# stormalex/minimap2_chaindp

Measured on AMD Instinct MI355X. Metric: chained anchors/sec (whole node), higher is better.
Workload: dtype int32

## Files before the change

### minimap2_chaindp_amd/csrc/chaindp_twin.hip

```cpp
#include <hip/hip_runtime.h>
#include <stdint.h>
#include <limits.h>
#include <stdio.h>
#include <stdlib.h>
#include <vector>
#include "chaindp_kernels.h"
#include "chaindp_wave.h"
#include "chaindp_lanes.h"

namespace chaindp {

#define TW_XY 0u
#define TW_PF 2048u
#define TW_V 3072u
#define TW_LUT_BYTES 512u
#define TW_ST_HALF 56u
#define TW_MK_HALF 260u
template <bool ONE_LUT> struct TwLayout {
	static constexpr bool HAS_XQ = !ONE_LUT;
	static constexpr uint32_t XQ = 3584u, XQ_HALF = 512u;
	static constexpr uint32_t LUT = ONE_LUT ? 3584u : XQ + 2u * XQ_HALF;
	static constexpr uint32_t LUT_HALF = ONE_LUT ? 0u : TW_LUT_BYTES;
	static constexpr uint32_t ST = LUT + (ONE_LUT ? 1u : 2u) * TW_LUT_BYTES;
	static constexpr uint32_t MK = ST + 2u * TW_ST_HALF;
	static constexpr uint32_t SP = MK + 2u * TW_MK_HALF;
	static constexpr uint32_t SP_HALF = ONE_LUT ? 0u : 64u;
	static constexpr uint32_t SP_OF_XQ = SP - XQ / 8u;
	static constexpr uint32_t KEY = SP + 128u;
	static constexpr uint32_t KEY_HALF = ONE_LUT ? 0u : 4u;
	static constexpr uint32_t BYTES = KEY + 8u;
	static_assert(ST % 8u == 0u && MK % 4u == 0u && KEY % 4u == 0u, "cold state is read as 64-bit words, marks and keys as 32-bit");
};
static_assert(TwLayout<true>::BYTES == 4864u && TwLayout<true>::BYTES <= 5120u, "one table: 32 workgroups per CU");
static_assert(TwLayout<false>::BYTES == 6400u, "two tables: 24 workgroups per CU");
template <bool SAMEGAP, bool ONE_LUT> struct TwWaves { static constexpr int N = !ONE_LUT ? 6 : SAMEGAP ? 8 : 7; };
#define TW_TILE 64
#define TW_RING 64
#define TW_QCH 8

__device__ __forceinline__ int tw_excl_max32(int v)
{
	v = max(v, __builtin_amdgcn_update_dpp(0, v, DPP_ROW_SHR(1), 0xf, 0xf, true));
	v = max(v, __builtin_amdgcn_update_dpp(0, v, DPP_ROW_SHR(2), 0xf, 0xf, true));
	v = max(v, __builtin_amdgcn_update_dpp(0, v, DPP_ROW_SHR(4), 0xf, 0xf, true));
	v = max(v, __builtin_amdgcn_update_dpp(0, v, DPP_ROW_SHR(8), 0xf, 0xf, true));
	int e = __builtin_amdgcn_update_dpp(0, v, DPP_ROW_SHR(1), 0xf, 0xf, true);
#if defined(__HIP_DEVICE_COMPILE__)
	asm("s_nop 1\n\tv_max_i32_dpp %0, %1, %0 row_bcast:15 row_mask:0xa bank_mask:0xf" : "+v"(e) : "v"(v));
#endif
	return e;
}
__device__ __forceinline__ int tw_incl_min32(int v)
{
	v = min(v, dpp_or_old<DPP_ROW_SHR(1), 0xf>(INT_MAX, v));
	v = min(v, dpp_or_old<DPP_ROW_SHR(2), 0xf>(INT_MAX, v));
	v = min(v, dpp_or_old<DPP_ROW_SHR(4), 0xf>(INT_MAX, v));
	v = min(v, dpp_or_old<DPP_ROW_SHR(8), 0xf>(INT_MAX, v));
	v = min(v, dpp_or_old<DPP_ROW_BCAST15, 0xa>(INT_MAX, v));
	return v;
}

__device__ __forceinline__ int tw_below_in_half(uint64_t m, bool hi_half)
{
	const int lo = (int)__builtin_amdgcn_mbcnt_lo((uint32_t)m, 0u);
	const int hi = (int)__builtin_amdgcn_mbcnt_hi((uint32_t)(m >> 32), 0u);
	return hi_half ? hi : lo;
}

__device__ __forceinline__ uint64_t tw_smear_halves(uint64_t m)
{
	uint32_t lo = 0, hi = 0;
#if defined(__HIP_DEVICE_COMPILE__)
	asm("s_cmp_lg_u32 %2, 0\n\ts_cselect_b32 %0, -1, 0\n\ts_cmp_lg_u32 %3, 0\n\ts_cselect_b32 %1, -1, 0"
	    : "=&s"(lo), "=&s"(hi) : "s"(TW_UNI((uint32_t)m)), "s"(TW_UNI((uint32_t)(m >> 32))) : "scc");
#endif
	return (uint64_t)hi << 32 | lo;
}

__device__ __forceinline__ uint64_t tw_last_or_lane0(uint64_t m)
{
	uint32_t lo = 0, hi = 0;
#if defined(__HIP_DEVICE_COMPILE__)
	asm("s_flbit_i32_b32 %0, %2\n\ts_flbit_i32_b32 %1, %3\n\ts_lshr_b32 %0, 0x80000000, %0\n\ts_lshr_b32 %1, 0x80000000, %1"
	    : "=&s"(lo), "=&s"(hi) : "s"(TW_UNI((uint32_t)m)), "s"(TW_UNI((uint32_t)(m >> 32))));
#endif
	return (uint64_t)hi << 32 | lo;
}

__device__ __forceinline__ uint32_t tw_both_halves(uint64_t m)
{
	uint32_t t = 0;
#if defined(__HIP_DEVICE_COMPILE__)
	asm("s_cmp_lg_u32 %1, 0\n\ts_cselect_b32 %0, %2, 0" : "=s"(t) : "s"(TW_UNI((uint32_t)m)), "s"(TW_UNI((uint32_t)(m >> 32))) : "scc");
#endif
	return t;
}

__device__ __forceinline__ uint64_t tw_below_first(uint64_t m, uint64_t b)
{
	const uint32_t blo = (uint32_t)b, bhi = (uint32_t)(b >> 32);
	const uint32_t klo = blo ? (blo & (0u - blo)) - 1u : 0xffffffffu, khi = bhi ? (bhi & (0u - bhi)) - 1u : 0xffffffffu;
	return m & ((uint64_t)khi << 32 | klo);
}

#define TW_HI31 0x8000000080000000ull

__device__ __forceinline__ uint64_t tw_above_first(uint64_t a, uint64_t b)
{
	uint32_t lo = 0, hi = 0;
#if defined(__HIP_DEVICE_COMPILE__)
	asm("s_sub_i32 %0, 0, %2\n\ts_sub_i32 %1, 0, %3" : "=&s"(lo), "=&s"(hi) : "s"(TW_UNI((uint32_t)b)), "s"(TW_UNI((uint32_t)(b >> 32))) : "scc");
#endif
	return a & ((uint64_t)hi << 32 | lo);
}

__device__ __forceinline__ void tw_st64_pf_lanes(uint64_t m, uint32_t a, uint32_t x, uint32_t y)
{
#if defined(__HIP_DEVICE_COMPILE__)
	tw_u32x2 t; t.x = x; t.y = y;
	uint64_t saved;
	asm volatile("s_and_saveexec_b64 %0, %1\n\tds_write_b64 %2, %3 offset:2048\n\ts_mov_b64 exec, %0"
	             : "=&s"(saved) : "s"(m), "v"(a), "v"(t) : "memory", "scc");
#endif
}
static_assert(TW_PF == 2048u, "tw_st64_pf_lanes writes the PF ring at DS offset 2048");


struct TwinArgs {
	Params par;
	const int64_t *off;
	const ulonglong2 *a;
	const unsigned long long *sumq;
	const uint16_t *lut;
	int lut_stride;
	const Unit *units;
	const UnitAux *aux;
	const unsigned long long *counters;
	int32_t *f, *p, *v;
	int32_t *first_child;
	uint8_t *flags;
	Unit *left;
	unsigned int *left_cnt;
	unsigned int *queue;
	const unsigned int *key_range;
	unsigned int *route;
	int two_tables;
	int force_left;
	int64_t total;
	unsigned long long *stamp;
};

struct TwinCold {
	int64_t next;
	int64_t base;
	uint64_t x_carry;
	int32_t rel0, room, read, tile0;
};

struct TwinHot {
	uint32_t S;
	uint32_t m4;
	uint32_t pc;
	uint32_t pend;
};
#define TW_CARRY 40u

#ifdef CHAINDP_TWIN_STAMPS
#define TW_STAMP(...) __VA_ARGS__
#else
#define TW_STAMP(...)
#endif
#if defined(CHAINDP_TWIN_STAMPS) && CHAINDP_TWIN_STAMPS == 2
#define TW_STAMP_A(...)
#define TW_STAMP_B(...) __VA_ARGS__
#elif defined(CHAINDP_TWIN_STAMPS) && CHAINDP_TWIN_STAMPS == 1
#define TW_STAMP_A(...) __VA_ARGS__
#define TW_STAMP_B(...)
#else
#define TW_STAMP_A(...)
#define TW_STAMP_B(...)
#endif
#if defined(CHAINDP_TWIN_STAMPS) && CHAINDP_TWIN_STAMPS == 3
#define TW_STAMP_C(...) __VA_ARGS__
#else
#define TW_STAMP_C(...)
#endif
#define TW_NOW() __builtin_amdgcn_s_memtime()

template <bool SAMEGAP, bool ONE_LUT>
__global__ __launch_bounds__(64) __attribute__((amdgpu_waves_per_eu(TwWaves<SAMEGAP, ONE_LUT>::N, TwWaves<SAMEGAP, ONE_LUT>::N))) void k_chain_twin(TwinArgs g)
{
	using L = TwLayout<ONE_LUT>;
	const int lane = threadIdx.x;
	const bool hi_half = lane >= 32;
	const int h = lane >> 5, hl = lane & 31;

	uint32_t L16 = ((uint32_t)hl + 1u) << 4;
	const uint32_t mkbase = L::MK + TW_MK_HALF * (uint32_t)h;
	const uint32_t curbase = L::XQ + L::XQ_HALF * (uint32_t)h;
	uint32_t c_mkbase = mkbase;
	uint32_t c_far = mkbase + 256u;
	uint32_t c_own = mkbase + ((uint32_t)hl << 2);
	uint32_t c_lut = ONE_LUT ? 0u : L::LUT + L::LUT_HALF * (uint32_t)h;
	uint32_t c_8h = (uint32_t)h << 3;
	uint32_t c_M = (uint32_t)g.par.max_dist_x;
	uint32_t c_bw = (uint32_t)g.par.bw;
	uint32_t c_cbw = c_M - 1u > c_bw ? c_M - 1u - c_bw : 0u;
	const uint32_t mdq = (uint32_t)(g.par.max_dist_x < g.par.max_dist_y ? g.par.max_dist_x : g.par.max_dist_y);
	uint32_t c_dqoff = c_M - mdq;
	int c_ms = g.par.max_skip;
	int c_min = INT_MIN;
	int c_Mout = hl == 31 ? g.par.max_dist_x : INT_MAX;
	uint32_t c_bwl = c_bw + c_lut;
	uint32_t c_cbwl = c_cbw - c_lut;
	constexpr uint32_t LUT_OFF = ONE_LUT ? L::LUT : 0u;
	TW_VREG(L16); TW_VREG(c_far); TW_VREG(c_own);
	if (!ONE_LUT) { TW_VREG(c_M); TW_VREG(c_ms); }
	if (!ONE_LUT) TW_VREG(c_lut);
	if (!SAMEGAP) TW_VREG(c_dqoff);
	TW_VREG(c_min); TW_VREG(c_Mout); TW_VREG(c_bwl); TW_VREG(c_cbwl);

	const uint64_t maxx = (uint64_t)(int64_t)g.par.max_dist_x;
	const uint32_t route = *g.route;
	if (ONE_LUT ? route == 1u || g.key_range[0] != g.key_range[1] || g.two_tables : route == 1u || route == 2u) return;
	const int64_t n_units = (int64_t)(uint32_t)g.counters[0];
	const int64_t n_single = (int64_t)(g.counters[0] >> 32);
	const bool short_units = (g.total - n_single) <= 512 * n_units;
	if (!short_units) {
		if (blockIdx.x == 0 && lane == 0) *g.left_cnt = 0xffffffffu;
		return;
	}
	if (blockIdx.x == 0 && lane == 0) *g.route = ONE_LUT ? 2u : 3u;
	const bool params_ok = g.lut != nullptr && !g.par.is_cdna && g.par.max_dist_x >= 1 && g.par.max_dist_y >= 0 &&
	                       ((uint64_t)(int64_t)g.par.max_dist_x + 1) * 129ull < (1ull << 31) && g.par.bw + 1 <= (int)TW_LUT_BYTES && g.force_left != 1;

	TwinHot u;
	u.S = 0; u.m4 = 0; u.pc = L::HAS_XQ ? curbase : 0u; u.pend = u.pc;
	uint64_t live_m = ~0ull;
	uint64_t contm = 0;
	const uint32_t st_addr = L::ST + TW_ST_HALF * (uint32_t)h;
#define TW_COLD (*TW_LDS(TwinCold, st_addr))
	const uint32_t xcd = blockIdx.x & 7u;
	const uint32_t n_halves = 2u * gridDim.x;
#ifndef TW_END_UNITS
#define TW_END_UNITS 16u
#define TW_PIECE 1u
#endif
	const uint32_t U1 = n_units > (long long)TW_END_UNITS * n_halves ? ((uint32_t)n_units - TW_END_UNITS * n_halves) & ~(8u * TW_QCH - 1u) : 0u;
	const uint32_t G1k = U1 / (8u * TW_QCH);
	auto grab = [&](uint32_t p, uint32_t &nx, uint32_t &ne) {
		if (p < G1k) { nx = (8u * p + xcd) * TW_QCH; ne = nx + TW_QCH; }
		else { nx = U1 + TW_PIECE * (8u * (p - G1k) + xcd); ne = nx + TW_PIECE; }
	};
	if (hl == 0) {
		uint32_t nx, ne;
		grab(((blockIdx.x >> 3) << 1) | (uint32_t)h, nx, ne);
		tw_st64(st_addr, nx, ne); tw_st64(st_addr + 8u, 0u, 0u);
		tw_st64(st_addr + 16u, 0u, 0u); tw_st64(st_addr + 24u, 0u, 0u);
		tw_st64(st_addr + 32u, 0u, (uint32_t)-TW_TILE);
		tw_st64(st_addr + TW_CARRY, 0xfffffffcu, 0u); tw_st64(st_addr + TW_CARRY + 8u, 0u, 0u);
		tw_st32(L::KEY + 4u * (uint32_t)h, -1);
	}
	wave_mem_fence();

	constexpr bool PF = !ONE_LUT;
	uint64_t nx0_x = 0, nx0_y = 0, nx1_x = 0, nx1_y = 0;
	int32_t pfu0 = -1, pfu1 = -1;

	TW_STAMP(unsigned long long st_t0 = 0; unsigned int st_service = 0, st_n_service = 0, st_n_fast = 0, st_flush = 0, st_unit = 0, st_n_unit = 0, st_head = 0, st_take = 0, st_tail = 0;)

	auto service = [&](uint64_t svc) {
#if defined(__HIP_DEVICE_COMPILE__)
		asm volatile("s_waitcnt vmcnt(0)" ::: "memory");
#endif
		wave_mem_fence();
		uint64_t retired = 0;
		for (int hs = 0; hs < 2; ++hs) {
			if (((svc >> (32 * hs)) & 1ull) == 0) continue;
			TW_STAMP_B(const unsigned long long th0 = g.stamp ? TW_NOW() : 0;)
			const uint64_t hm = hs ? 0xffffffff00000000ull : 0x00000000ffffffffull;
			const uint32_t sa = L::ST + TW_ST_HALF * (uint32_t)hs, keya = L::KEY + L::KEY_HALF * (uint32_t)hs;
			const uint32_t mkb = L::MK + TW_MK_HALF * (uint32_t)hs, lutb = L::LUT + L::LUT_HALF * (uint32_t)hs;
			const uint32_t curb = L::XQ + L::XQ_HALF * (uint32_t)hs, spb = L::SP + L::SP_HALF * (uint32_t)hs;
			const tw_u32x2 cw0 = tw_ld64(sa), cw1 = tw_ld64(sa + 8u), cw2 = tw_ld64(sa + 16u), cw3 = tw_ld64(sa + 24u), cw4 = tw_ld64(sa + 32u);
			int64_t c_next = (int64_t)((uint64_t)TW_UNI(cw0.y) << 32 | TW_UNI(cw0.x));
			int64_t c_base = (int64_t)((uint64_t)TW_UNI(cw1.y) << 32 | TW_UNI(cw1.x));
			uint64_t c_xcarry = (uint64_t)TW_UNI(cw2.y) << 32 | TW_UNI(cw2.x);
			int c_rel0 = (int)TW_UNI(cw3.x), c_room = (int)TW_UNI(cw3.y), c_read = (int)TW_UNI(cw4.x), c_tile0 = (int)TW_UNI(cw4.y);
			auto tile_cnt = [&]() -> int {
				const uint32_t pe = TW_UNI(__builtin_amdgcn_readlane((int)u.pend, 32 * hs));
				if constexpr (L::HAS_XQ) return (int)((pe - curb) >> 3);
				else return pe < mkb ? 0 : (int)((pe - mkb) >> 2) + 1 - c_tile0;
			};
			const int cnt_prev = tile_cnt();
			const int slow_h = (int)TW_UNI((uint32_t)tw_ld32(sa + TW_CARRY + 12u));
			const uint32_t cur_key = TW_UNI((uint32_t)tw_ld32(keya));
			const int tile_prev = c_tile0, rel0_prev = c_rel0;
			const int64_t base_prev = c_base;
			bool live = true;
			const uint32_t nx0 = (uint32_t)c_next, ne0 = (uint32_t)((uint64_t)c_next >> 32);
			tw_u32x4 rec0 = {0u, 0u, 0u, 0u}, aux0 = {0u, 0u, 0u, 0u}, rec1 = {0u, 0u, 0u, 0u};
			const bool rec0_ok = nx0 < ne0 && (int64_t)nx0 < n_units;
			const bool rec1_ok = PF && rec0_ok && nx0 + 1u < ne0 && (int64_t)nx0 + 1 < n_units;
			if (rec0_ok) { rec0 = *TW_CONST(tw_u32x4, g.units + nx0); aux0 = *TW_CONST(tw_u32x4, g.aux + nx0); }
			if (rec1_ok) rec1 = *TW_CONST(tw_u32x4, g.units + nx0 + 1u);

			auto take_tile = [&](const uint64_t an_x, const uint64_t an_y) -> int {
				const int i_lane = c_tile0 + lane;
				const bool have = i_lane < c_room;
				uint64_t xp;
				{
					uint32_t lo = (uint32_t)wave_shift_up1((int)(uint32_t)an_x, 0), hi = (uint32_t)wave_shift_up1((int)(uint32_t)(an_x >> 32), 0);
					if (lane == 0) { lo = (uint32_t)c_xcarry; hi = (uint32_t)(c_xcarry >> 32); }
					xp = (uint64_t)hi << 32 | lo;
				}
				const bool stop = !have || (i_lane > 0 && an_x - xp > maxx);
				const uint64_t stop_m = __builtin_amdgcn_ballot_w64(stop);
				const int cnt = stop_m ? __builtin_ctzll(stop_m) : TW_TILE;
				c_xcarry = readlane_u64(an_x, 63);
				if constexpr (L::HAS_XQ) { u.pc = TW_SEL(hm, curb, u.pc); u.pend = TW_SEL(hm, curb + ((uint32_t)cnt << 3), u.pend); }
				else u.pend = TW_SEL(hm, mkb + ((uint32_t)(c_tile0 + cnt - 1) << 2), u.pend);
				if (cnt == 0) return 0;
				wave_mem_fence();
				if (lane < cnt) {
					const int sp = span_of_hi((uint32_t)(an_y >> 32));
					tw_st64((((uint32_t)i_lane & 127u) << 4 | (uint32_t)hs << 3) + TW_XY, (uint32_t)an_x + 1u, (uint32_t)an_y + 1u);
					if constexpr (L::HAS_XQ) {
						tw_st64(curb + ((uint32_t)lane << 3), (uint32_t)an_x, (uint32_t)an_y);
						tw_st8(spb + (uint32_t)lane, sp - 1);
					} else tw_st8((((uint32_t)i_lane & 63u) << 1 | (uint32_t)hs) + L::SP, sp - 1);
					g.first_child[c_base + i_lane] = NO_CHILD;
				}
				wave_mem_fence();
				if constexpr (PF) {
					if (cnt == TW_TILE && c_tile0 + TW_TILE < c_room) {
						uint64_t rx = 0, ry = 0;
						if (i_lane + TW_TILE < c_room) { const ulonglong2 t = g.a[c_base + i_lane + TW_TILE]; rx = t.x; ry = t.y; }
						if (hs) { nx1_x = rx; nx1_y = ry; pfu1 = -1; } else { nx0_x = rx; nx0_y = ry; pfu0 = -1; }
					}
				}
				return cnt;
			};

			bool goes_on = cnt_prev == TW_TILE && c_tile0 + TW_TILE < c_room;
			if (goes_on && (slow_h * 8 > c_tile0 + TW_TILE || g.force_left == 2)) {
				if (lane == 0) {
					Unit un; un.start = (int64_t)((uint64_t)c_base | (uint64_t)(uint32_t)(c_tile0 + TW_TILE) << 32); un.read = c_read; un.len = c_room;
					g.left[atomicAdd(g.left_cnt, 1u)] = un;
				}
				goes_on = false;
			}
			if (goes_on) {
				c_tile0 += TW_TILE;
				uint64_t nt_x = 0, nt_y = 0;
				if constexpr (PF) { nt_x = hs ? nx1_x : nx0_x; nt_y = hs ? nx1_y : nx0_y; }
				else if (c_tile0 + lane < c_room) { const ulonglong2 t = g.a[c_base + c_tile0 + lane]; nt_x = t.x; nt_y = t.y; }
				if (take_tile(nt_x, nt_y) == 0) goes_on = false;
			}
			TW_STAMP_B(if (g.stamp) st_take += (unsigned int)(TW_NOW() - th0);)
			TW_STAMP_A(const unsigned long long tf0 = g.stamp ? TW_NOW() : 0;)
			if (cnt_prev > 0) {
				const int i_lane = tile_prev + lane;
				const bool have = lane < cnt_prev;
				const int64_t gi = base_prev + i_lane;
				int fi = 0, p4 = -4;
				if (have) {
					const tw_u32x2 pf = tw_ld64((((uint32_t)i_lane & 63u) << 4 | (uint32_t)hs << 3) + TW_PF);
					p4 = (int)pf.x; fi = (int)pf.y + 1;
				}
				const int pi = p4 >> 2;
				int val = fi, ptr = have ? pi : -1;
				const bool ext = ptr >= 0 && ptr < tile_prev;
				int vext = 0;
				if (ext) {
					vext = tw_ld32((((uint32_t)ptr & 63u) << 3 | (uint32_t)hs << 2) + TW_V);
					val = max(val, vext & 0x7fffffff);
					ptr = -1;
				}
				const bool ext_self = ext && vext < 0;
				for (int r = 0; r < 6; ++r) {
					if (__builtin_amdgcn_ballot_w64(ptr >= tile_prev) == 0) break;
					const int src = (ptr >= tile_prev ? ptr - tile_prev : lane) << 2;
					const int pv = __builtin_amdgcn_ds_bpermute(src, val);
					const int pp = __builtin_amdgcn_ds_bpermute(src, ptr);
					if (ptr >= tile_prev) { val = max(val, pv); ptr = pp; }
				}
				const bool self = val >= g.par.min_sc || pi >= 0;
				const int srcp = (pi >= tile_prev ? pi - tile_prev : lane) << 2;
				const int pself_in = __builtin_amdgcn_ds_bpermute(srcp, self ? 1 : 0);
				const bool pred_self = ext ? ext_self : pself_in != 0;
				wave_mem_fence();
				if (have) tw_st32((((uint32_t)i_lane & 63u) << 3 | (uint32_t)hs << 2) + TW_V, val | (self ? INT_MIN : 0));
				wave_mem_fence();
				if (have) {
					g.f[gi] = fi;
					g.p[gi] = pi < 0 ? -1 : pi + rel0_prev;
					g.v[gi] = val;
					int maybe_first = 0;
					if (pi >= 0 && !pred_self) { atomicMin(&g.first_child[base_prev + pi], rel0_prev + i_lane); maybe_first = 4; }
					g.flags[gi] = (uint8_t)((self ? 2 : 0) | maybe_first | (val >= g.par.min_sc ? 8 : 0) | (fi < val ? 16 : 0));
				}
			}
			TW_STAMP_A(if (g.stamp) st_flush += (unsigned int)(TW_NOW() - tf0);)
			TW_STAMP_A(const unsigned long long tu0 = g.stamp ? TW_NOW() : 0;)
			TW_STAMP_A(if (g.stamp && !goes_on) ++st_n_unit;)
			bool have_rec = rec0_ok;
			const bool rec0_used = !goes_on;
			uint32_t cur_key_now = cur_key;
			while (!goes_on && live) {
				uint32_t nx = (uint32_t)c_next, ne = (uint32_t)((uint64_t)c_next >> 32);
				if (nx >= ne) {
					uint32_t q0 = 0;
					if (lane == 0) q0 = atomicAdd(g.queue + 64u * xcd, 1u);
					grab(TW_UNI(q0), nx, ne);
					have_rec = false;
				}
				if ((int64_t)nx >= n_units) {
					c_next = (int64_t)((uint64_t)ne << 32 | nx); live = false;
					if constexpr (L::HAS_XQ) { u.pc = TW_SEL(hm, curb, u.pc); u.pend = TW_SEL(hm, curb, u.pend); }
					else u.pend = TW_SEL(hm, 0u, u.pend);
					break;
				}
				TW_STAMP_C(const unsigned long long tc0 = g.stamp ? TW_NOW() : 0;)
				if (!have_rec) { rec0 = *TW_CONST(tw_u32x4, g.units + nx); aux0 = *TW_CONST(tw_u32x4, g.aux + nx); }
				have_rec = false;
				TW_STAMP_C(if (g.stamp) { asm volatile("" :: "s"(rec0.x), "s"(aux0.x)); st_head += (unsigned int)(TW_NOW() - tc0); })
				c_next = (int64_t)((uint64_t)ne << 32 | (nx + 1u));
				Unit un;
				un.start = (int64_t)((uint64_t)rec0.y << 32 | rec0.x); un.read = (int32_t)rec0.z; un.len = (int32_t)rec0.w;
				if (!params_ok || (aux0.z & 1u) || g.par.n_segs > 1 || (ONE_LUT && cur_key_now != 0xffffffffu && aux0.y != cur_key_now)) {
					if (lane == 0) g.left[atomicAdd(g.left_cnt, 1u)] = un;
					continue;
				}
				c_base = un.start; c_rel0 = (int)aux0.x; c_room = un.len; c_read = un.read; c_tile0 = 0;
				uint64_t tl_x = 0, tl_y = 0;
				TW_STAMP_C(const unsigned long long tc1 = g.stamp ? TW_NOW() : 0;)
				TW_STAMP_C(if (g.stamp && PF && (hs ? pfu1 : pfu0) == (int32_t)c_base) ++st_n_unit;)
				if (PF && (hs ? pfu1 : pfu0) == (int32_t)c_base) { tl_x = hs ? nx1_x : nx0_x; tl_y = hs ? nx1_y : nx0_y; }
				else if (lane < c_room) { const ulonglong2 t = g.a[c_base + lane]; tl_x = t.x; tl_y = t.y; }
				if constexpr (PF) { if (hs) pfu1 = -1; else pfu0 = -1; }
				TW_STAMP_C(if (g.stamp) { asm volatile("" :: "v"(tl_x), "v"(tl_y)); asm volatile("s_waitcnt vmcnt(0)" ::: "memory"); st_take += (unsigned int)(TW_NOW() - tc1); })
				TW_STAMP_C(const unsigned long long tc2 = g.stamp ? TW_NOW() : 0;)
				wave_mem_fence();
				if (aux0.y != cur_key_now) {
					const uint2 *src = (const uint2*)(g.lut + (int64_t)c_read * g.lut_stride);
					for (int k = lane; k * 4 <= g.par.bw; k += 64) {
						const uint2 t = src[k];
						const uint32_t w = (t.x & 0xffu) | (t.x >> 8 & 0xff00u) | (t.y << 16 & 0xff0000u) | (t.y << 8 & 0xff000000u);
						tw_st32(lutb + ((uint32_t)k << 2), (int)w);
					}
					cur_key_now = aux0.y;
					if (lane == 0) tw_st32(keya, (int)cur_key_now);
				}
				const uint32_t x_none = (uint32_t)__builtin_amdgcn_readlane((int)(uint32_t)tl_x, 0) - (uint32_t)maxx - 1u;
				for (int k = lane; k < 128; k += 64) tw_st64(((uint32_t)k << 4 | (uint32_t)hs << 3) + TW_XY, x_none, 0u);
				for (int k = lane; k < 65; k += 64) tw_st32(mkb + ((uint32_t)k << 2), -1);
				wave_mem_fence();
				c_xcarry = 0;
				if (lane == 0) tw_st32(sa + TW_CARRY + 12u, 0);
				if (take_tile(tl_x, tl_y) > 0) goes_on = true;
				TW_STAMP_C(if (g.stamp) { st_tail += (unsigned int)(TW_NOW() - tc2); ++st_unit; })
			}
			if (PF && live) {
				const int cnt_now = tile_cnt();
				const uint32_t nxn = (uint32_t)c_next, nen = (uint32_t)((uint64_t)c_next >> 32);
				if (!(cnt_now == TW_TILE && c_tile0 + TW_TILE < c_room) && (hs ? pfu1 : pfu0) < 0 && nxn < nen && (int64_t)nxn < n_units &&
				    ((nxn == nx0 && rec0_ok && !rec0_used) || (nxn == nx0 + 1u && rec1_ok))) {
					const tw_u32x4 rn = nxn == nx0 ? rec0 : rec1;
					const int32_t st = (int32_t)rn.x, ln = (int32_t)rn.w;
					uint64_t rx = 0, ry = 0;
					if (lane < ln) { const ulonglong2 t = g.a[(int64_t)st + lane]; rx = t.x; ry = t.y; }
					if (hs) { nx1_x = rx; nx1_y = ry; pfu1 = st; } else { nx0_x = rx; nx0_y = ry; pfu0 = st; }
				}
			}
			TW_STAMP_A(if (g.stamp) st_unit += (unsigned int)(TW_NOW() - tu0);)
			if (live) {
				const uint32_t i = (uint32_t)c_tile0;
				u.S = TW_SEL(hm, (i - 1u) << 4 | (uint32_t)hs << 3, u.S); u.m4 = TW_SEL(hm, ((i - 1u) << 2) + mkb, u.m4);
			} else retired |= hm;
			if (lane == 0) {
				tw_st64(sa, (uint32_t)c_next, (uint32_t)((uint64_t)c_next >> 32)); tw_st64(sa + 8u, (uint32_t)c_base, (uint32_t)((uint64_t)c_base >> 32));
				tw_st64(sa + 16u, (uint32_t)c_xcarry, (uint32_t)(c_xcarry >> 32)); tw_st64(sa + 24u, (uint32_t)c_rel0, (uint32_t)c_room);
				tw_st64(sa + 32u, (uint32_t)c_read, (uint32_t)c_tile0);
			}
		}
		wave_mem_fence();
		live_m &= ~retired;
		contm &= ~svc;
	};

	auto slow_tail = [&](uint64_t D, uint32_t a_cur, int nskip_after) -> uint64_t {
		const uint64_t giveup = ~D & contm;
		const int vlast = __builtin_amdgcn_ds_bpermute(((h << 5) + 31) << 2, nskip_after);
		wave_mem_fence();
		const tw_u32x2 cur = tw_ld64(a_cur);
		if (__builtin_amdgcn_inverse_ballot_w64(D)) {
			u.m4 += 4u;
			u.S = ((u.m4 - c_mkbase) << 2) | c_8h;
			if constexpr (L::HAS_XQ) u.pc += 8u;
		} else {
			if (hl == 0) {
				tw_st64(st_addr + TW_CARRY, cur.x, cur.y);
				tw_st32(st_addr + TW_CARRY + 8u, vlast);
				tw_st32(st_addr + TW_CARRY + 12u, tw_ld32(st_addr + TW_CARRY + 12u) + 1);
			}
			u.S -= 512u;
		}
		contm = ~D & ~giveup & live_m;
		if (__builtin_expect(giveup != 0, 0)) {
			if (__builtin_amdgcn_inverse_ballot_w64(giveup)) {
				wave_mem_fence();
				if (hl == 0) {
					const TwinCold c = TW_COLD;
					Unit un; un.start = (int64_t)((uint64_t)c.base | (uint64_t)(uint32_t)c.tile0 << 32); un.read = c.read; un.len = c.room;
					g.left[atomicAdd(g.left_cnt, 1u)] = un;
				}
				u.pc = curbase; u.pend = L::HAS_XQ ? curbase : 0u;
			}
			return giveup;
		}
		return 0;
	};

	TW_STAMP(if (g.stamp) st_t0 = TW_NOW();)
	service(~0ull);
	bool force_general = false;
	while (live_m != 0) {
		wave_mem_fence();
		uint64_t svc = 0;
		if (__builtin_expect(contm == 0 && live_m == ~0ull && !force_general, 1)) {
			if constexpr (ONE_LUT) {
				uint64_t B, D = 0;
				bool tile_end = false;
				int npass = 1;
				if constexpr (L::HAS_XQ) {
					const int n0 = (int)(TW_UNI(__builtin_amdgcn_readlane((int)u.pend, 0)) - TW_UNI(__builtin_amdgcn_readlane((int)u.pc, 0))) >> 3;
					const int n1 = (int)(TW_UNI(__builtin_amdgcn_readlane((int)u.pend, 32)) - TW_UNI(__builtin_amdgcn_readlane((int)u.pc, 32))) >> 3;
					npass = max(min(n0, n1), 1);
				} else {
					const int n0 = (int)(TW_UNI(__builtin_amdgcn_readlane((int)u.pend, 0)) - TW_UNI(__builtin_amdgcn_readlane((int)u.m4, 0))) >> 2;
					const int n1 = (int)(TW_UNI(__builtin_amdgcn_readlane((int)u.pend, 32)) - TW_UNI(__builtin_amdgcn_readlane((int)u.m4, 32))) >> 2;
					npass = max(min(n0, n1), 1);
				}
				const uint32_t ms0 = (uint32_t)max(g.par.max_skip, 0);
				u.S += 16u;
				for (;;) {
					const uint32_t S1 = u.S;
					const uint32_t t0 = S1 - L16;
					const tw_u32x2 xy = tw_ld64((t0 & 0x7f8u) + TW_XY);
					const tw_u32x2 cur = tw_ld64(L::HAS_XQ ? u.pc : (S1 & 0x7f8u) + TW_XY);
	#if defined(__HIP_DEVICE_COMPILE__)
					__builtin_amdgcn_sched_barrier(0);
	#endif
					const tw_u32x2 pf = tw_ld64((t0 & 0x3f8u) + TW_PF);
					uint32_t a_cur = S1 & 0x3f8u;
					TW_OPAQUE(a_cur);
					const int spm1 = tw_ld_u8(L::HAS_XQ ? (u.pc >> 3) + L::SP_OF_XQ : (a_cur >> 3) + L::SP);
	#ifdef TW_EXP_PAD
					for (int k = 0; k < TW_EXP_PAD; ++k) { uint32_t pad; asm volatile("v_max3_u32 %0, %1, %1, %1" : "=v"(pad) : "v"(c_far)); }
	#endif
					const uint32_t drm1 = L::HAS_XQ ? cur.x - xy.x : tw_sub_m1(cur.x, xy.x), dqm1 = L::HAS_XQ ? cur.y - xy.y : tw_sub_m1(cur.y, xy.y);
					const uint32_t ddl = ONE_LUT ? tw_absdiff(drm1, dqm1) : tw_sad(drm1, dqm1, c_lut);
					const uint32_t dqs = SAMEGAP ? dqm1 : __builtin_elementwise_add_sat(dqm1, c_dqoff);
					const uint32_t m3 = max(max(drm1, dqs), ddl + c_cbwl);
					const uint64_t okm = TW_ULT(m3, c_M);
					const uint32_t dst = TW_SEL(okm, min(u.m4 - pf.x, c_far), c_far);
					tw_st32(dst, (int)u.m4);
					wave_mem_fence();
					const int tj = tw_ld32(c_own);
					const int lutv = tw_ld_i8(min(ddl, c_bwl) + LUT_OFF);
	#if defined(__HIP_DEVICE_COMPILE__)
					__builtin_amdgcn_sched_barrier(0);
	#endif
					const int sc0 = min(min((int)dqm1, (int)drm1), spm1);
					const int sc = TW_SEL(okm, sc0 + (int)pf.y + lutv, c_min);
					const int excl = max(tw_excl_max32(sc), spm1);
					const uint64_t A = TW_SGT(sc, excl);
					B = TW_EQ(tj, u.m4) & okm & ~A;
					const uint32_t blo = (uint32_t)B, bhi = (uint32_t)(B >> 32);
					if (__builtin_expect(tw_above_first(A, B) != 0, 0)) { force_general = true; break; }
					{
						const uint32_t wp = TW_SEL(A, u.m4 - c_own, 0xfffffffcu);
						const int wf = max(excl, sc);
						tw_st64_pf_lanes(tw_last_or_lane0(A), a_cur, wp, (uint32_t)wf);
					}
					const uint32_t nlo = (uint32_t)__builtin_popcount(blo), nhi = (uint32_t)__builtin_popcount(bhi);
					if (__builtin_expect(min(nlo, nhi) <= ms0, 0)) {
						const uint64_t OUT = TW_SGE(drm1, c_Mout);
						D = tw_smear_halves(OUT | (nlo > ms0 ? 0x00000000ffffffffull : 0ull) | (nhi > ms0 ? 0xffffffff00000000ull : 0ull));
						if (__builtin_expect(tw_both_halves(D) == 0, 0)) break;
					}
					u.m4 += 4u; u.S += 16u;
					if constexpr (L::HAS_XQ) u.pc += 8u;
					TW_STAMP(if (g.stamp) ++st_n_fast;)
					if (__builtin_expect(--npass <= 0, 0)) { tile_end = true; break; }
					wave_mem_fence();
				}
				const uint32_t a_cur = u.S & 0x3f8u;
				u.S -= 16u;
				if (!force_general && !tile_end) {
					svc = slow_tail(D, a_cur + TW_PF, tw_below_in_half(B, hi_half) + (int)__builtin_amdgcn_inverse_ballot_w64(B));
				}
			} else {
				uint64_t B, X, tile;
				int cB;
				uint32_t a_cur;
				for (;;) {
					const uint32_t S1 = u.S + 16u;
					const uint32_t t0 = S1 - L16;
					const tw_u32x2 xy = tw_ld64((t0 & 0x7f8u) + TW_XY);
					const tw_u32x2 cur = tw_ld64(u.pc);
	#if defined(__HIP_DEVICE_COMPILE__)
					__builtin_amdgcn_sched_barrier(0);
	#endif
					const tw_u32x2 pf = tw_ld64((t0 & 0x3f8u) + TW_PF);
					const int spm1 = tw_ld_u8((u.pc >> 3) + L::SP_OF_XQ);
					const uint32_t drm1 = cur.x - xy.x, dqm1 = cur.y - xy.y;
					const uint32_t ddl = tw_sad(drm1, dqm1, c_lut);
					const uint32_t dqs = SAMEGAP ? dqm1 : __builtin_elementwise_add_sat(dqm1, c_dqoff);
					const uint32_t m3 = max(max(drm1, dqs), ddl + c_cbwl);
					const uint64_t okm = TW_ULT(m3, c_M);
					const uint32_t dst = TW_SEL(okm, min(u.m4 - pf.x, c_far), c_far);
					tw_st32(dst, (int)u.m4);
					wave_mem_fence();
					const int tj = tw_ld32(c_own);
					const int lutv = tw_ld_i8(min(ddl, c_bwl) + LUT_OFF);
	#if defined(__HIP_DEVICE_COMPILE__)
					__builtin_amdgcn_sched_barrier(0);
	#endif
					const int sc0 = min(min((int)dqm1, (int)drm1), spm1);
					const int sc = TW_SEL(okm, sc0 + (int)pf.y + lutv, c_min);
					const int excl = max(tw_excl_max32(sc), spm1);
					const uint64_t A = TW_SGT(sc, excl);
					B = TW_EQ(tj, u.m4) & okm & ~A;
					const uint64_t OUT = TW_SGE(drm1, c_Mout);
					cB = tw_below_in_half(B, hi_half);
					tile = 0; X = 0; a_cur = 0;
					if (__builtin_expect((TW_SGT(cB, 0) & A) != 0, 0)) { force_general = true; break; }
					a_cur = S1 & 0x3f8u;
					{
						const uint32_t wp = TW_SEL(A, u.m4 - c_own, 0xfffffffcu);
						const int wf = TW_SEL(A, sc, spm1);
						if (__builtin_amdgcn_inverse_ballot_w64(tw_last_or_lane0(A))) tw_st64(a_cur + TW_PF, wp, (uint32_t)wf);
					}
					X = (TW_SGE(cB, c_ms) & B) | OUT;
					if (__builtin_expect(tw_both_halves(X) == 0, 0)) break;
					u.m4 += 4u; u.S = S1;
					u.pc += 8u; tile = TW_SGE(u.pc, u.pend);
					TW_STAMP(if (g.stamp) ++st_n_fast;)
					if (__builtin_expect(tile != 0, 0)) break;
					wave_mem_fence();
				}
				if (!force_general && tile == 0) {
					svc = slow_tail(tw_smear_halves(X), a_cur + TW_PF, cB + (int)__builtin_amdgcn_inverse_ballot_w64(B));
				}
			}
		} else {
			force_general = false;
			const uint32_t t0 = u.S + 16u - L16;
			const uint32_t xcur = ((((u.m4 - c_mkbase) + 4u) << 2) & 0x7f8u) | c_8h;
			const tw_u32x2 xy = tw_ld64((t0 & 0x7f8u) + TW_XY);
			const tw_u32x2 pf = tw_ld64((t0 & 0x3f8u) + TW_PF);
			const tw_u32x2 cur = tw_ld64(L::HAS_XQ ? u.pc : xcur + TW_XY);
			const int spm1 = tw_ld_u8(L::HAS_XQ ? (u.pc >> 3) + L::SP_OF_XQ : ((xcur >> 3) & 0x7fu) + L::SP);
			const uint64_t first = ~contm;
			const tw_u32x2 carry = tw_ld64(st_addr + TW_CARRY);
			const int maxf = TW_SEL(first, spm1, (int)carry.y);
			const uint32_t maxj4 = TW_SEL(first, 0xfffffffcu, carry.x);
			const int nskip0 = TW_SEL(first, 0, tw_ld32(st_addr + TW_CARRY + 8u));
			const uint32_t kb4 = TW_SEL(first, 0u, 128u);
			const uint32_t drm1 = L::HAS_XQ ? cur.x - xy.x : tw_sub_m1(cur.x, xy.x), dqm1 = L::HAS_XQ ? cur.y - xy.y : tw_sub_m1(cur.y, xy.y);
			const uint32_t ddl = ONE_LUT ? tw_absdiff(drm1, dqm1) : tw_sad(drm1, dqm1, c_lut);
			const uint32_t dqs = SAMEGAP ? dqm1 : __builtin_elementwise_add_sat(dqm1, c_dqoff);
			const uint32_t m3 = max(max(drm1, dqs), ddl + c_cbwl);
			const uint64_t okm = TW_ULT(m3, c_M) & ~(contm & TW_HI31) & live_m;
			const int sc0 = min(min((int)dqm1, (int)drm1), spm1);
			const int lutv = tw_ld_i8(min(ddl, c_bwl) + LUT_OFF);
			const uint32_t dst = TW_SEL(okm, min(u.m4 - pf.x, c_far), c_far);
			tw_st32(dst, (int)u.m4);
			wave_mem_fence();
			const int tj = tw_ld32(c_own + kb4);
			const int sc = TW_SEL(okm, sc0 + (int)pf.y + lutv, c_min);
			const int excl = max(tw_excl_max32(sc), maxf);
			const uint64_t A = TW_SGT(sc, excl);
			const uint64_t B = TW_EQ(tj, u.m4) & okm & ~A;
			const uint64_t OUT = TW_SGE(drm1, c_M);
			const int cB = tw_below_in_half(B, hi_half), cA = tw_below_in_half(A, hi_half);
			const int isA = (int)__builtin_amdgcn_inverse_ballot_w64(A), isB = (int)__builtin_amdgcn_inverse_ballot_w64(B);
			const uint64_t inter = TW_SGT(cB, 0) & A;
			uint64_t brk, Ap;
			int nskip_after;
			if (inter == 0) {
				nskip_after = max(nskip0 - cA - isA, 0) + cB + isB;
				brk = TW_SGT(nskip_after, c_ms) & B;
				Ap = A;
			} else {
				const int Sk = nskip0 + cB + isB - cA - isA;
				nskip_after = Sk - min(tw_incl_min32(Sk), 0);
				brk = TW_SGT(nskip_after, c_ms) & B;
				Ap = tw_below_first(A, brk);
			}
			const uint32_t a_cur = (xcur & 0x3f8u) + TW_PF;
			{
				const uint32_t wp = TW_SEL(Ap, u.m4 - c_own - kb4, maxj4);
				const int wf = TW_SEL(Ap, sc, maxf);
				if (__builtin_amdgcn_inverse_ballot_w64(tw_last_or_lane0(Ap))) tw_st64(a_cur, wp, (uint32_t)wf);
			}
			const uint64_t D = tw_smear_halves(brk | (OUT & TW_HI31) | ~live_m);
			svc = slow_tail(D, a_cur, nskip_after);
		}
		svc |= tw_smear_halves((L::HAS_XQ ? TW_SGE(u.pc, u.pend) : TW_SGE(u.m4, u.pend)) & live_m & ~contm);
		if (__builtin_expect(svc != 0, 0)) {
			TW_STAMP(const unsigned long long ts = g.stamp ? TW_NOW() : 0;)
			service(svc & live_m);
			TW_STAMP(if (g.stamp) { st_service += (unsigned int)(TW_NOW() - ts); ++st_n_service; })
		}
	}
	TW_STAMP(if (g.stamp && lane == 0) {
		unsigned long long *o = g.stamp + 12 * (size_t)blockIdx.x;
		o[0] = TW_NOW() - st_t0; o[1] = st_service; o[2] = st_flush; o[3] = st_unit; o[4] = st_n_service; o[5] = st_n_fast; o[6] = st_n_unit; o[7] = 1; o[8] = st_head; o[9] = st_take; o[10] = st_tail;
	})
#undef TW_COLD
}

size_t twin_lds_bytes(bool one_table) { return one_table ? TwLayout<true>::BYTES : TwLayout<false>::BYTES; }

int twin_max_wg_per_cu(bool samegap, bool one_table)
{
	const int lds_wg = one_table ? 32 : 24;
	const int waves = one_table ? (samegap ? TwWaves<true, true>::N : TwWaves<false, true>::N)
	                            : (samegap ? TwWaves<true, false>::N : TwWaves<false, false>::N);
	return 4 * waves < lds_wg ? 4 * waves : lds_wg;
}

template <bool ONE_LUT>
static hipError_t launch_twin_layout(hipStream_t st, TwinArgs g, int64_t max_units, int cus, unsigned int *d_queue)
{
	const bool samegap = g.par.max_dist_y >= g.par.max_dist_x;
	const int max_wg = twin_max_wg_per_cu(samegap, ONE_LUT);
	int64_t blocks = (max_units + 2 * TW_QCH - 1) / (2 * TW_QCH);
	static const int wg_env = getenv("CHAINDP_TWIN_WG_PER_CU") ? atoi(getenv("CHAINDP_TWIN_WG_PER_CU")) : 0;
	const int64_t cap = (int64_t)cus * (wg_env >= 1 && wg_env <= max_wg ? wg_env : max_wg);
	if (blocks > cap) blocks = cap;
	if (blocks < 1) blocks = 1;
	blocks = (blocks + 7) & ~(int64_t)7;
	{
		const hipError_t e = hipMemsetD32Async((hipDeviceptr_t)d_queue, (int)(2 * blocks / 8), 8 * 64, st);
		if (e != hipSuccess) return e;
	}
	static unsigned long long *d_stamp = nullptr;
	const bool stamp = getenv("CHAINDP_TWIN_STAMP") != nullptr;
	if (stamp && !d_stamp && hipMalloc((void**)&d_stamp, (size_t)cap * 96) != hipSuccess) d_stamp = nullptr;
	g.stamp = stamp ? d_stamp : nullptr;
	if (g.stamp) (void)hipMemsetAsync(d_stamp, 0, (size_t)blocks * 96, st);
	{
		hipFuncAttributes fa;
		const void *fn = samegap ? (const void*)k_chain_twin<true, ONE_LUT> : (const void*)k_chain_twin<false, ONE_LUT>;
		const hipError_t e = hipFuncGetAttributes(&fa, fn);
		if (e != hipSuccess) return e;
		if (fa.sharedSizeBytes != 0) return hipErrorInvalidConfiguration;
	}
	if (samegap) hipLaunchKernelGGL((k_chain_twin<true, ONE_LUT>), dim3((unsigned)blocks), dim3(64), TwLayout<ONE_LUT>::BYTES, st, g);
	else hipLaunchKernelGGL((k_chain_twin<false, ONE_LUT>), dim3((unsigned)blocks), dim3(64), TwLayout<ONE_LUT>::BYTES, st, g);
	if (g.stamp) {
		std::vector<unsigned long long> hb((size_t)blocks * 12);
		if (hipStreamSynchronize(st) == hipSuccess && hipMemcpy(hb.data(), d_stamp, hb.size() * 8, hipMemcpyDeviceToHost) == hipSuccess) {
			double tot = 0, svc = 0, flush = 0, unit = 0, nsvc = 0, nfast = 0, nunit = 0, nb = 0, head = 0, take = 0, tail = 0;
			for (int64_t b = 0; b < blocks; ++b) if (hb[(size_t)b * 12 + 7]) {
				const unsigned long long *o = &hb[(size_t)b * 12];
				tot += o[0]; svc += o[1]; flush += o[2]; unit += o[3]; nsvc += o[4]; nfast += o[5]; nunit += o[6]; head += o[8]; take += o[9]; tail += o[10]; ++nb;
			}
			if (nb > 0) fprintf(stderr, "[twin stamp raw] sums over waves: head %.0f take %.0f tail %.0f unit %.0f n_unit %.0f (build 3: ticks until the record / the first tile / the rest of a unit switch; switches; first tiles requested ahead)\n", head, take, tail, unit, nunit);
			if (nb > 0) fprintf(stderr, "[twin stamp] %.0f waves, %.0f ticks each: service %.1f%% (%.0f calls, %.0f ticks each: cold state and decisions %.0f, next tile %.0f, flush %.0f, "
			                "unit switch %.0f (%.0f switches, %.0f ticks each), first anchor and cold state back %.0f), passes %.0f (%.0f ticks each, everything else included)\n",
			        nb, tot / nb, 100.0 * svc / tot, nsvc, svc / (nsvc > 0 ? nsvc : 1), head / (nsvc > 0 ? nsvc : 1), take / (nsvc > 0 ? nsvc : 1), flush / (nsvc > 0 ? nsvc : 1),
			        unit / (nsvc > 0 ? nsvc : 1), nunit, unit / (nunit > 0 ? nunit : 1), tail / (nsvc > 0 ? nsvc : 1), nfast, (tot - svc) / (nfast > 0 ? nfast : 1));
		}
	}
	return hipGetLastError();
}

hipError_t launch_chain_twin(hipStream_t st, const Params &par, int64_t max_units, const int64_t *d_off, const void *d_a,
                             const unsigned long long *d_sumq, const uint16_t *d_lut, int lut_stride, const Unit *d_units,
                             const unsigned long long *d_counters, int32_t *d_f, int32_t *d_p, int32_t *d_v,
                             int32_t *d_first_child, uint8_t *d_flags, Unit *d_left, unsigned int *d_left_cnt, int force_left, int64_t total,
                             const UnitAux *d_unit_aux, const unsigned int *d_key_range, unsigned int *d_route, unsigned int *d_queue, int two_tables)
{
	if (max_units <= 0) return hipSuccess;
	if (!d_unit_aux || !d_key_range || !d_route || !d_queue) return hipErrorInvalidValue;
	int dev = 0, cus = 256;
	if (hipGetDevice(&dev) == hipSuccess) (void)hipDeviceGetAttribute(&cus, hipDeviceAttributeMultiprocessorCount, dev);
	TwinArgs g;
	g.par = par; g.off = d_off; g.a = (const ulonglong2*)d_a; g.sumq = d_sumq; g.lut = d_lut; g.lut_stride = lut_stride;
	g.units = d_units; g.aux = d_unit_aux; g.counters = d_counters; g.f = d_f; g.p = d_p; g.v = d_v; g.first_child = d_first_child; g.flags = d_flags;
	g.left = d_left; g.left_cnt = d_left_cnt; g.queue = d_queue; g.key_range = d_key_range; g.route = d_route; g.two_tables = two_tables != 0;
	g.force_left = force_left; g.total = total; g.stamp = nullptr;
	hipError_t e = launch_twin_layout<true>(st, g, max_units, cus, d_queue);
	if (e == hipSuccess) e = launch_twin_layout<false>(st, g, max_units, cus, d_queue);
	return e;
}

}
```

Measured before the change: 21.82 billion.

## Fuse fast-path loop exit checks into a single scalar key comparison

Restructures the ONE_LUT fast chaining loop so each iteration folds three checks into one scalar key: the above-first conflict test, the max_skip popcount test and the pass-count test. The key is built by a new inline-asm helper, leaving one uniform branch per step, and the detailed exit handling runs only after the inner do-while leaves. Early-tile lanes are forced into the exit mask E so npass is capped, and the out-of-range test now uses c_M masked to the top lane of each half instead of a per-lane c_Mout, which frees that register. It aims to cut scalar branch and compare work on the latency-bound serial DP step, but it adds rollback bookkeeping (undoing m4/S on exit) and the HAS_XQ pc increment is dropped, which risks correctness on that layout.

```diff
diff --git a/minimap2_chaindp_amd/csrc/chaindp_twin.hip b/minimap2_chaindp_amd/csrc/chaindp_twin.hip
--- a/minimap2_chaindp_amd/csrc/chaindp_twin.hip
+++ b/minimap2_chaindp_amd/csrc/chaindp_twin.hip
@@ -114,6 +114,18 @@
 	return a & ((uint64_t)hi << 32 | lo);
 }
 
+__device__ __forceinline__ uint32_t tw_exit_key(uint64_t a, uint64_t b, uint32_t k, uint64_t &ia)
+{
+#if defined(__HIP_DEVICE_COMPILE__)
+	uint32_t lo, hi;
+	asm("s_sub_i32 %0, 0, %2\n\ts_sub_i32 %1, 0, %3" : "=&s"(lo), "=&s"(hi) : "s"(TW_UNI((uint32_t)b)), "s"(TW_UNI((uint32_t)(b >> 32))) : "scc");
+	asm("s_and_b64 %1, %2, %3\n\ts_cselect_b32 %0, 0, %0" : "+s"(k), "=&s"(ia) : "s"(a), "s"((uint64_t)hi << 32 | lo) : "scc");
+#else
+	ia = tw_above_first(a, b); k = ia ? 0u : k;
+#endif
+	return k;
+}
+
 __device__ __forceinline__ void tw_st64_pf_lanes(uint64_t m, uint32_t a, uint32_t x, uint32_t y)
 {
 #if defined(__HIP_DEVICE_COMPILE__)
@@ -215,10 +227,10 @@
 	uint32_t c_cbwl = c_cbw - c_lut;
 	constexpr uint32_t LUT_OFF = ONE_LUT ? L::LUT : 0u;
 	TW_VREG(L16); TW_VREG(c_far); TW_VREG(c_own);
-	if (!ONE_LUT) { TW_VREG(c_M); TW_VREG(c_ms); }
+	if (!ONE_LUT) { TW_VREG(c_M); TW_VREG(c_ms); TW_VREG(c_Mout); }
 	if (!ONE_LUT) TW_VREG(c_lut);
 	if (!SAMEGAP) TW_VREG(c_dqoff);
-	TW_VREG(c_min); TW_VREG(c_Mout); TW_VREG(c_bwl); TW_VREG(c_cbwl);
+	TW_VREG(c_min); TW_VREG(c_bwl); TW_VREG(c_cbwl);
 
 	const uint64_t maxx = (uint64_t)(int64_t)g.par.max_dist_x;
 	const uint32_t route = *g.route;
@@ -530,7 +542,8 @@
 		uint64_t svc = 0;
 		if (__builtin_expect(contm == 0 && live_m == ~0ull && !force_general, 1)) {
 			if constexpr (ONE_LUT) {
-				uint64_t B, D = 0;
+				uint64_t B, D = 0, I, E = 0;
+				uint32_t drx;
 				bool tile_end = false;
 				int npass = 1;
 				if constexpr (L::HAS_XQ) {
@@ -538,64 +551,85 @@
 					const int n1 = (int)(TW_UNI(__builtin_amdgcn_readlane((int)u.pend, 32)) - TW_UNI(__builtin_amdgcn_readlane((int)u.pc, 32))) >> 3;
 					npass = max(min(n0, n1), 1);
 				} else {
-					const int n0 = (int)(TW_UNI(__builtin_amdgcn_readlane((int)u.pend, 0)) - TW_UNI(__builtin_amdgcn_readlane((int)u.m4, 0))) >> 2;
-					const int n1 = (int)(TW_UNI(__builtin_amdgcn_readlane((int)u.pend, 32)) - TW_UNI(__builtin_amdgcn_readlane((int)u.m4, 32))) >> 2;
+					const uint32_t m0 = TW_UNI(__builtin_amdgcn_readlane((int)u.m4, 0)), m1 = TW_UNI(__builtin_amdgcn_readlane((int)u.m4, 32));
+					const int n0 = (int)(TW_UNI(__builtin_amdgcn_readlane((int)u.pend, 0)) - m0) >> 2;
+					const int n1 = (int)(TW_UNI(__builtin_amdgcn_readlane((int)u.pend, 32)) - m1) >> 2;
 					npass = max(min(n0, n1), 1);
+					const int e0 = 31 - ((int)(m0 - L::MK) >> 2), e1 = 31 - ((int)(m1 - L::MK - TW_MK_HALF) >> 2);
+					if (e0 > 0) { E |= 0x00000000ffffffffull; npass = min(npass, e0); }
+					if (e1 > 0) { E |= 0xffffffff00000000ull; npass = min(npass, e1); }
 				}
 				const uint32_t ms0 = (uint32_t)max(g.par.max_skip, 0);
+				uint32_t P = (uint32_t)npass + ms0;
 				u.S += 16u;
 				for (;;) {
-					const uint32_t S1 = u.S;
-					const uint32_t t0 = S1 - L16;
-					const tw_u32x2 xy = tw_ld64((t0 & 0x7f8u) + TW_XY);
-					const tw_u32x2 cur = tw_ld64(L::HAS_XQ ? u.pc : (S1 & 0x7f8u) + TW_XY);
+					uint32_t key;
+					do {
+						const uint32_t S1 = u.S;
+						const uint32_t t0 = S1 - L16;
+						const tw_u32x2 xy = tw_ld64((t0 & 0x7f8u) + TW_XY);
+						const tw_u32x2 cur = tw_ld64(L::HAS_XQ ? u.pc : (S1 & 0x7f8u) + TW_XY);
 	#if defined(__HIP_DEVICE_COMPILE__)
-					__builtin_amdgcn_sched_barrier(0);
+						__builtin_amdgcn_sched_barrier(0);
 	#endif
-					const tw_u32x2 pf = tw_ld64((t0 & 0x3f8u) + TW_PF);
-					uint32_t a_cur = S1 & 0x3f8u;
-					TW_OPAQUE(a_cur);
-					const int spm1 = tw_ld_u8(L::HAS_XQ ? (u.pc >> 3) + L::SP_OF_XQ : (a_cur >> 3) + L::SP);
+						const tw_u32x2 pf = tw_ld64((t0 & 0x3f8u) + TW_PF);
+						uint32_t a_cur = S1 & 0x3f8u;
+						TW_OPAQUE(a_cur);
+						const int spm1 = tw_ld_u8(L::HAS_XQ ? (u.pc >> 3) + L::SP_OF_XQ : (a_cur >> 3) + L::SP);
 	#ifdef TW_EXP_PAD
-					for (int k = 0; k < TW_EXP_PAD; ++k) { uint32_t pad; asm volatile("v_max3_u32 %0, %1, %1, %1" : "=v"(pad) : "v"(c_far)); }
+						for (int k = 0; k < TW_EXP_PAD; ++k) { uint32_t pad; asm volatile("v_max3_u32 %0, %1, %1, %1" : "=v"(pad) : "v"(c_far)); }
 	#endif
-					const uint32_t drm1 = L::HAS_XQ ? cur.x - xy.x : tw_sub_m1(cur.x, xy.x), dqm1 = L::HAS_XQ ? cur.y - xy.y : tw_sub_m1(cur.y, xy.y);
-					const uint32_t ddl = ONE_LUT ? tw_absdiff(drm1, dqm1) : tw_sad(drm1, dqm1, c_lut);
-					const uint32_t dqs = SAMEGAP ? dqm1 : __builtin_elementwise_add_sat(dqm1, c_dqoff);
-					const uint32_t m3 = max(max(drm1, dqs), ddl + c_cbwl);
-					const uint64_t okm = TW_ULT(m3, c_M);
-					const uint32_t dst = TW_SEL(okm, min(u.m4 - pf.x, c_far), c_far);
-					tw_st32(dst, (int)u.m4);
+						const uint32_t drm1 = L::HAS_XQ ? cur.x - xy.x : tw_sub_m1(cur.x, xy.x), dqm1 = L::HAS_XQ ? cur.y - xy.y : tw_sub_m1(cur.y, xy.y);
+						drx = drm1;
+						const uint32_t ddl = ONE_LUT ? tw_absdiff(drm1, dqm1) : tw_sad(drm1, dqm1, c_lut);
+						const uint32_t dqs = SAMEGAP ? dqm1 : __builtin_elementwise_add_sat(dqm1, c_dqoff);
+						const uint32_t m3 = max(max(drm1, dqs), ddl + c_cbwl);
+						const uint64_t okm = TW_ULT(m3, c_M);
+						const uint32_t dst = TW_SEL(okm, min(u.m4 - pf.x, c_far), c_far);
+						tw_st32(dst, (int)u.m4);
+						wave_mem_fence();
+						const int tj = tw_ld32(c_own);
+						const int lutv = tw_ld_i8(min(ddl, c_bwl) + LUT_OFF);
+	#if defined(__HIP_DEVICE_COMPILE__)
+						__builtin_amdgcn_sched_barrier(0);
+	#endif
+						const int sc0 = min(min((int)dqm1, (int)drm1), spm1);
+						const int sc = TW_SEL(okm, sc0 + (int)pf.y + lutv, c_min);
+						const int excl = max(tw_excl_max32(sc), spm1);
+						const uint64_t A = TW_SGT(sc, excl);
+						B = TW_EQ(tj, u.m4) & okm & ~A;
+						{
+							const uint32_t wp = TW_SEL(A, u.m4 - c_own, 0xfffffffcu);
+							const int wf = max(excl, sc);
+							tw_st64_pf_lanes(tw_last_or_lane0(A), a_cur, wp, (uint32_t)wf);
+						}
+#ifdef TW_EXP_SPAD
+						for (int k = 0; k < TW_EXP_SPAD; ++k) { uint32_t pad; asm volatile("s_xor_b32 %0, %0, %0" : "=s"(pad) :: "scc"); }
+#endif
+						u.m4 += 4u; u.S += 16u;
+						--P;
+						const uint64_t BE = B | E;
+						uint32_t nmin = min((uint32_t)__builtin_popcount((uint32_t)BE), (uint32_t)__builtin_popcount((uint32_t)(BE >> 32)));
+	#if defined(__HIP_DEVICE_COMPILE__)
+						asm("" : "+s"(nmin));
+	#endif
+						key = tw_exit_key(A, B, min(nmin, P), I);
+						TW_STAMP(if (g.stamp && key > ms0) ++st_n_fast;)
+						wave_mem_fence();
+					} while (__builtin_expect(key > ms0, 1));
+					if (I != 0) { force_general = true; break; }
+					const uint32_t nlo = (uint32_t)__builtin_popcount((uint32_t)B), nhi = (uint32_t)__builtin_popcount((uint32_t)(B >> 32));
+					if (min(nlo, nhi) <= ms0) {
+						const uint64_t OUT = TW_SGE(drx, c_M) & TW_HI31;
+						D = tw_smear_halves(OUT | (nlo > ms0 ? 0x00000000ffffffffull : 0ull) | (nhi > ms0 ? 0xffffffff00000000ull : 0ull));
+						if (tw_both_halves(D) == 0) break;
+					}
+					TW_STAMP(if (g.stamp) ++st_n_fast;)
+					if (P <= ms0) { tile_end = true; break; }
 					wave_mem_fence();
-					const int tj = tw_ld32(c_own);
-					const int lutv = tw_ld_i8(min(ddl, c_bwl) + LUT_OFF);
-	#if defined(__HIP_DEVICE_COMPILE__)
-					__builtin_amdgcn_sched_barrier(0);
-	#endif
-					const int sc0 = min(min((int)dqm1, (int)drm1), spm1);
-					const int sc = TW_SEL(okm, sc0 + (int)pf.y + lutv, c_min);
-					const int excl = max(tw_excl_max32(sc), spm1);
-					const uint64_t A = TW_SGT(sc, excl);
-					B = TW_EQ(tj, u.m4) & okm & ~A;
-					const uint32_t blo = (uint32_t)B, bhi = (uint32_t)(B >> 32);
-					if (__builtin_expect(tw_above_first(A, B) != 0, 0)) { force_general = true; break; }
-					{
-						const uint32_t wp = TW_SEL(A, u.m4 - c_own, 0xfffffffcu);
-						const int wf = max(excl, sc);
-						tw_st64_pf_lanes(tw_last_or_lane0(A), a_cur, wp, (uint32_t)wf);
-					}
-					const uint32_t nlo = (uint32_t)__builtin_popcount(blo), nhi = (uint32_t)__builtin_popcount(bhi);
-					if (__builtin_expect(min(nlo, nhi) <= ms0, 0)) {
-						const uint64_t OUT = TW_SGE(drm1, c_Mout);
-						D = tw_smear_halves(OUT | (nlo > ms0 ? 0x00000000ffffffffull : 0ull) | (nhi > ms0 ? 0xffffffff00000000ull : 0ull));
-						if (__builtin_expect(tw_both_halves(D) == 0, 0)) break;
-					}
-					u.m4 += 4u; u.S += 16u;
-					if constexpr (L::HAS_XQ) u.pc += 8u;
-					TW_STAMP(if (g.stamp) ++st_n_fast;)
-					if (__builtin_expect(--npass <= 0, 0)) { tile_end = true; break; }
-					wave_mem_fence();
-				}
+				}
+				TW_OPAQUE(u.S); TW_OPAQUE(u.m4);
+				if (!tile_end) { u.m4 -= 4u; u.S -= 16u; }
 				const uint32_t a_cur = u.S & 0x3f8u;
 				u.S -= 16u;
 				if (!force_general && !tile_end) {
```

Result: faster. 22.80 billion, median of 6 (+4.5%).
